# GBATZOLIS/conditional_score_diffusion

Hardware: AMD Instinct MI355X
Metric: images/sec for 1000-step PC sampling, ddpm_paired_SR3 score net of celebA_SR3_160 (BASELINE configs[1]), 160x160 (higher is better)
Workload: dtype f16x3 (every operand carried as hi + lo fp16 = 22 significand bits, 3 MFMAs per product, f32 accumulate; f32-class: the per-op test tolerance is the f32 kernel's, network error 1.9e-6 vs the reference); 1 GPU; BASELINE configs[1]: celebA_SR3_160 (ddpm_paired_SR3, nf=96, ch_mult (1,1,2,2,3,3), attn 20/10/5), 1000-step PC (reverse_diffusion + langevin, snr 0.15), batch 64 per GPU, random-init weights, synthetic LR inputs; images_per_gpu=64, global_batch=64, noise=on-device Philox4x32-10, precision_mode=fp16x3

## Files before the change

conditional_score_diffusion_amd/_lib.py:

```python
import ctypes
import os
import subprocess
import sys

_HERE = os.path.dirname(os.path.abspath(__file__))
LIB_PATH = os.environ.get('CSD_LIB_PATH', os.path.join(_HERE, 'libcsd_hip.so'))
CSRC = os.path.join(_HERE, 'csrc')

MAX_LEVELS = 8
MAX_ATTN = 8

ACT_IDS = {'none': 0, 'swish': 1, 'relu': 2, 'lrelu': 3, 'elu': 4}
PREC_IDS = {'fp32': 0, 'f32': 0, 'fp16x3': 1, 'fp16': 2, 'fp16f8': 3}


class UNetConfig(ctypes.Structure):
    _fields_ = [('arch', ctypes.c_int32), ('nf', ctypes.c_int32), ('n_levels', ctypes.c_int32),
                ('ch_mult', ctypes.c_int32 * MAX_LEVELS), ('num_res_blocks', ctypes.c_int32),
                ('n_attn', ctypes.c_int32), ('attn_resolutions', ctypes.c_int32 * MAX_ATTN),
                ('image_size', ctypes.c_int32), ('x_channels', ctypes.c_int32),
                ('y_channels', ctypes.c_int32), ('out_channels', ctypes.c_int32),
                ('resamp_with_conv', ctypes.c_int32), ('conditional', ctypes.c_int32),
                ('centered', ctypes.c_int32), ('act', ctypes.c_int32), ('precision', ctypes.c_int32),
                ('skip_rescale', ctypes.c_int32), ('progressive', ctypes.c_int32), ('progressive_input', ctypes.c_int32),
# ... 83 lines not shown
    'csd_reverse_diffusion_step_ex': (_i, [_vp, _vp, _vp, _vp, _f, _f, _f, _f, _i, _f, _f, _i, _i64, _vp]),
    'csd_row_norms': (_i, [_vp, _vp, _i, _i64, _vp]),
    'csd_affine_noise_step': (_i, [_vp, _vp, _vp, _vp, _f, _f, _f, _i64, _vp]),
    'csd_linear': (_i, [_vp, _vp, _vp, _vp, _i, _i, _i, _i, _vp]),
    'csd_fourier_embedding': (_i, [_vp, _vp, _vp, _i, _i, _vp]),
    'csd_axpby': (_i, [_vp, _vp, _vp, _f, _f, _f, _f, _i64, _vp]),
    'csd_bias_add_nchw': (_i, [_vp, _vp, _vp, _i, _i, _i64, _i, _i, _vp]),
    'csd_randn': (_i, [_vp, _i64, _u64, _u64, _vp]),
    'csd_scale_rows': (_i, [_vp, _vp, _vp, _i, _i, _i64, _vp]),
    'csd_groupnorm_scratch_bytes': (_sz, [_i, _i, _i, _i]),
    'csd_groupnorm_act': (_i, [_vp, _vp, _vp, _vp, _i, _i, _i, _i, _i, _f, _i, _vp, _vp]),
    'csd_conv_scratch_bytes': (_sz, [_i, _i, _i, _i, _i, _i, _i]),
    'csd_conv2d': (_i, [_vp, _vp, _vp, _vp, _i, _i, _i, _i, _i, _i, _i, _i, _i, _i, _vp, _vp]),
    'csd_attention_scratch_bytes': (_sz, [_i, _i, _i, _i]),
    'csd_attention': (_i, [_vp, _vp, _vp, _vp, _i, _i, _i, _i, _vp, _vp]),
    'csd_fir_pyr_conv_scratch_bytes': (_sz, [_i, _i]),
    'csd_fir_pyr_conv': (_i, [_vp, _vp, _vp, _vp, _vp, _i, _i, _i, _i, _i, _vp, _f, _vp, _vp]),
    'csd_upfirdn2d': (_i, [_vp, _vp, _vp, _i, _i, _i, _i, _i, _i, _i, _i, _i, _i, _i, _i, _i, _i, _vp]),
    'csd_fused_bias_act': (_i, [_vp, _vp, _vp, _vp, _i64, _i, _i64, _i, _i, _f, _f, _vp]),
    'csd_nearest_up2': (_i, [_vp, _vp, _i, _i, _i, _i, _vp]),
    'csd_timestep_embedding': (_i, [_vp, _vp, _i, _i, _vp]),
    'csd_conv_wgrad_scratch_bytes': (_sz, [_i, _i, _i, _i, _i, _i, _i, _i]),
    'csd_conv2d_wgrad': (_i, [_vp, _vp, _vp, _i, _i, _i, _i, _i, _i, _i, _i, _i, _vp, _vp]),
    'csd_groupnorm_act_backward': (_i, [_vp, _vp, _vp, _vp, _vp, _vp, _vp, _i, _i, _i, _i, _i, _f, _i, _vp]),
    'csd_attention_backward_scratch_bytes': (_sz, [_i, _i, _i, _i]),
    'csd_attention_backward': (_i, [_vp, _vp, _vp, _vp, _vp, _vp, _vp, _i, _i, _i, _i, _vp, _vp]),
    'csd_bgemm': (_i, [_vp, _vp, _vp, _i, _i, _i, _i64, _i64, _i64, _i64, _i64, _i64, _i, _i64, _i64, _i64, _f, _vp]),
    'csd_sum_inner': (_i, [_vp, _vp, _i64, _i64, _vp]),
    'csd_sum_rows': (_i, [_vp, _vp, _i, _i, _vp]),
    'csd_act': (_i, [_vp, _vp, _vp, _i, _i64, _vp]),
    'csd_mul': (_i, [_vp, _vp, _vp, _i64, _vp]),
    'csd_conv3x3_block_scratch_bytes': (_sz, [_i, _i]),
    'csd_conv3x3_block': (_i, [_vp, _vp, _vp, _vp, _vp, _vp, _vp, _i, _vp, _f, _vp, _vp, _i, _i, _i, _i, _i, _i, _i, _vp, _vp]),
    'csd_conv2d_ex': (_i, [_vp, _vp, _vp, _vp, _i, _i, _i, _i, _i, _i, _i, _i, _i, _i, _i, _vp, _vp]),
    'csd_conv2d_wgrad_ex': (_i, [_vp, _vp, _vp, _i, _i, _i, _i, _i, _i, _i, _i, _i, _i, _vp, _vp]),
    'csd_groupnorm_nhwc_scratch_bytes': (_sz, [_i, _i, _i]),
    'csd_groupnorm_act_nhwc': (_i, [_vp, _vp, _vp, _vp, _vp, _vp, _i, _i, _i, _i, _f, _i, _vp, _vp]),
    'csd_groupnorm_act_backward_nhwc': (_i, [_vp, _vp, _vp, _vp, _vp, _vp, _vp, _vp, _vp, _i, _i, _i, _i, _i, _i, _vp, _vp]),
    'csd_bias_add_nhwc': (_i, [_vp, _vp, _vp, _i, _i, _i, _vp]),
    'csd_sum_pixels_scratch_bytes': (_sz, [_i, _i, _i]),
    'csd_sum_pixels_nhwc': (_i, [_vp, _vp, _i, _i, _i, _vp, _vp]),
    'csd_zero_insert_odd_nhwc': (_i, [_vp, _vp, _i, _i, _i, _i, _vp]),
    'csd_sumpool2_nhwc': (_i, [_vp, _vp, _i, _i, _i, _i, _vp]),
    'csd_attention_nhwc': (_i, [_vp, _vp, _i, _i, _i, _vp]),
    'csd_attention_nhwc_prec': (_i, [_vp, _vp, _i, _i, _i, _i, _vp]),
    'csd_attention_backward_nhwc': (_i, [_vp, _vp, _vp, _i, _i, _i, _vp, _vp]),
    'csd_adam_step': (_i, [_vp, _vp, _vp, _vp, _vp, _vp, _i64, _i, _f, _f, _f, _f, _f, _f, _f, _vp]),
    'csd_global_norm_scratch_bytes': (_sz, []),
    'csd_global_norm': (_i, [_vp, _vp, _i64, _vp, _vp]),
    'csd_ema_update': (_i, [_vp, _vp, _i64, _f, _vp]),
    'csd_dropout': (_i, [_vp, _vp, _vp, _f, _u64, _u64, _i64, _vp]),
    'csd_pf_ode_state': (_i, [_vp, _vp, _vp, _vp, _i, _i64, _vp]),
    'csd_pf_ode_scratch_bytes': (_sz, [_i, _i64]),
    'csd_pf_ode_rhs': (_i, [_vp, _vp, _vp, _vp, _i64, _vp, _vp, _vp, _i, _i64, _vp, _vp]),
}


def lib():
    global _lib
    if _lib is None:
        if not os.path.exists(LIB_PATH):
            raise RuntimeError(
                'libcsd_hip.so not found at %s - run `python -c "import __graft_entry__ as g; g.build()"` '
                '(or `make -C %s`). There is no CPU fallback.' % (LIB_PATH, CSRC))
        l = ctypes.CDLL(LIB_PATH)
        for name, (res, args) in SIGNATURES.items():
# ... 63 lines not shown
```

conditional_score_diffusion_amd/csrc/common.h:

```cpp
#pragma once
#include <hip/hip_runtime.h>
#include <stdint.h>
#include <stdio.h>
#include <string>

#include "../../include/csd.h"

#ifdef CSD_TUNE
#define CSD_TUNE_ENV(name) getenv(name)
#else
#define CSD_TUNE_ENV(name) (static_cast<const char*>(nullptr))
#endif

namespace csd {

void set_error(const char* fmt, ...);
const char* get_error();

#define CSD_CHECK_HIP(expr)                                                         \
  do {                                                                              \
    hipError_t _e = (expr);                                                         \
    if (_e != hipSuccess) {                                                         \
      csd::set_error("%s:%d: %s -> %s", __FILE__, __LINE__, #expr, hipGetErrorString(_e)); \
      return CSD_ERR_HIP;                                                           \
// ... 113 lines not shown
int conv_pack_weight(const ConvPlan& p, const float* w, int layout, int cin_src, int cout_src, int cout_off,
                     float* wpack, hipStream_t s);
int conv_launch(const ConvPlan& p, const ConvArgs& a, hipStream_t s);

bool conv16_supported(const ConvPlan& p);
int conv16_kcs(int ns, int cin);
int conv16_plan_tiles(ConvPlan* p, int ns, int kcs = 1, bool lc = false);
size_t conv16_packed_bytes(const ConvPlan& p, int ns);
int conv16_pack_weight(const ConvPlan& p, int ns, const float* w, int layout, int cin_src, int cout_src,
                       int cout_off, void* wpack, hipStream_t s);
int conv16_launch(const ConvPlan& p, int ns, const ConvArgs& a, hipStream_t s, bool in16 = false);
bool conv16q_supported(const ConvPlan& p, int ns);
size_t conv16q_packed_bytes(const ConvPlan& p, int ns);
int conv16q_pack_weight(const ConvPlan& p, int ns, const float* w, int layout, int cin_src, int cout_src, int cout_off,
                        void* wpack, hipStream_t s);
int conv16q_plan_tiles(ConvPlan* p, int ns);
bool conv16q_up4_supported(const ConvPlan& p, int ns);
bool conv16q_up4_stats_ok(const ConvPlan& p);
size_t conv16q_up4_packed_bytes(const ConvPlan& p, int ns);
int conv16q_pack_weight_up4(const ConvPlan& p, int ns, const float* w, void* wpack, hipStream_t s);
int conv16q_launch(const ConvPlan& p, int ns, const ConvArgs& a, hipStream_t s, bool raw = false);
bool convff_supported(const ConvPlan& p, int ns);
size_t convff_packed_bytes(const ConvPlan& p, int ns);
int convff_pack_weight(const ConvPlan& p, int ns, const float* w, int layout, int cin_src, int cout_src, int cout_off,
                       void* wpack, hipStream_t s);
int convff_plan_tiles(ConvPlan* p, int ns);
bool convff_pipelined(const ConvPlan& p, int ns);
int convff_launch(const ConvPlan& p, int ns, const ConvArgs& a, hipStream_t s);
bool pw16_supported(const ConvPlan& p, int ns);
size_t pw16_packed_bytes(const ConvPlan& p, int ns);
int pw16_pack_weight(const ConvPlan& p, int ns, const float* w, int layout, int cin_src, int cout_src, int cout_off,
                     void* wpack, hipStream_t s);
int pw16_launch(const ConvPlan& p, int ns, const ConvArgs& a, hipStream_t s);
bool pw16_taps_supported(int cin, int cout, int ns);
int pw16_taps_cout(int cout);
int pw16_pack_weight_taps(const ConvPlan& p, int ns, const float* w, int cout, void* wpack, hipStream_t s);
int tapsum_launch(const float* part, const float* bias, const float* res, float* out, int B, int H, int W, int cout, int nchw,
                  float out_scale, hipStream_t s);
bool stem_supported(int Cx, int Cy, int Cout, int S, int ns);
size_t stem_packed_bytes(int Cout, int ns);
int stem_pack_weight(const float* w, int Cin, int Cout, int ns, void* wpack, hipStream_t s);
int stem_tiles_per_image(int S);
int stem_launch(const float* x, const float* y, const float* y_noise, float y_sigma, const void* wpack, const float* bias, float* out,
                double* stats, int B, int Cx, int Cy, int Cout, int S, int centered, int ns, hipStream_t s);
int gn_fused16_groups(int HW, int C0, int C1, int G);
int gn_fused16_launch(const float* src0, const float* src1, int C0, int C1, const float* gamma, const float* beta, float eps,
                      void* hi, void* lo, int B, int HW, int G, int act, hipStream_t s, int f8, float* nscale = nullptr,
                      float* nshift = nullptr);
int gn_apply16_launch(const float* src0, const float* src1, int C0, int C1, const float* nscale, const float* nshift,
                      void* hi, void* lo, int B, int HW, int act, hipStream_t s, int f8 = 0);
static inline int precision_ns(int precision) {
  return (precision == CSD_PREC_F16X3 || precision == CSD_PREC_F16F8) ? 2 : (precision == CSD_PREC_F16 ? 1 : 0);
}

struct GNPlan {
  int B, HW, C0, C1, G, nchunk;
};
size_t gn_partial_bytes(const GNPlan& p);
int gn_plan(GNPlan* p, int B, int HW, int C0, int C1, int G);
int gn_stats_launch(const GNPlan& p, const float* src0, const float* src1, double* partial,
                    hipStream_t s, int per_channel = 0);
int gn_finalize_launch(const GNPlan& p, const double* partial, const float* gamma, const float* beta,
                       float eps, float* nscale, float* nshift, hipStream_t s, float* rs = nullptr, float* ms = nullptr);
int gn_finalize_tiles_launch(const double* p0, int tpi0, int C0, const double* p1, int tpi1, int C1, int B, int HW, int G,
                             const float* gamma, const float* beta, float eps, float* nscale, float* nshift,
                             hipStream_t s);
// ... 78 lines not shown
```

conditional_score_diffusion_amd/csrc/conv_pw16.hip:

```cpp
#include <stdlib.h>
#include <string.h>

#include "common.h"

namespace csd {

typedef _Float16 half8_t __attribute__((ext_vector_type(8)));
typedef float floatx4 __attribute__((ext_vector_type(4)));
typedef float v4f_t __attribute__((ext_vector_type(4)));
typedef unsigned int uint4_t __attribute__((ext_vector_type(4)));

#define PW_THREADS 256
#define PW_NTL 6
#define PW_WSCALE 256.0f
#ifndef PW_DEPTH
#define PW_DEPTH 2
#endif

struct PwKArgs {
  ConvArgs a;
  int C0, C1, Cout;
  int npix;
  int hw;
  int ks;
  int ntiles;
};

__device__ __forceinline__ float4 pw_gload4(const float* p) {
  const v4f_t v = *(const __attribute__((address_space(1))) v4f_t*)(p);
  return make_float4(v.x, v.y, v.z, v.w);
}

template <int NS, int MTP, int OCC>
__global__ __launch_bounds__(PW_THREADS, OCC) void pw16_kernel(const float* __restrict__ g_src0,
                                                          const float* __restrict__ g_src1,
                                                          const char* __restrict__ g_wpack, const PwKArgs k) {
  extern __shared__ __attribute__((aligned(16))) char smem[];
  constexpr int WPIX = MTP * 16;
  constexpr int TPIX = 4 * WPIX;
  const int tid = threadIdx.x;
  const int lane = tid & 63;
  const int wave = tid >> 6;
  const int l16 = lane & 15;
  const int kq = lane >> 4;
  const int ng = blockIdx.y;
  const int Cin = k.C0 + k.C1;

  const int wbytes = k.ks * PW_NTL * NS * 1024;
  float* const lds_bias = reinterpret_cast<float*>(smem + wbytes);
  const int col_base = ng * (PW_NTL * 16) + kq * 4;

  const int nt_mine = (k.ntiles - (int)blockIdx.x + (int)gridDim.x - 1) / (int)gridDim.x;
  const int total = nt_mine * k.ks;
  const bool has_norm = k.a.nscale != nullptr;
  const bool has_res = k.a.res != nullptr;
  const bool has_act = k.a.act == CSD_ACT_SWISH;
  const int ntl = min(PW_NTL, (k.Cout - (int)blockIdx.y * (PW_NTL * 16) + 15) / 16);

  constexpr int D = MTP == 1 ? 4 : PW_DEPTH;
  float4 raw[D][MTP][2];
  constexpr bool PFN = MTP == 1;
  float4 nsc[PFN ? D : 1][MTP][2], nsh[PFN ? D : 1][MTP][2];
  floatx4 acc[MTP][PW_NTL];
#pragma unroll
  for (int j = 0; j < MTP; ++j)
#pragma unroll
    for (int nt = 0; nt < PW_NTL; ++nt) acc[j][nt] = floatx4{0.f, 0.f, 0.f, 0.f};

  int l_tile = blockIdx.x, l_kk = 0, l_it = 0;
  int c_tile = blockIdx.x, c_kk = 0;

  auto issue = [&](float4 (&dst)[MTP][2], float4 (&dsc)[MTP][2], float4 (&dsh)[MTP][2]) {
    if (l_it < total) {
      const int kb = l_kk * 32;
      const bool s1 = kb >= k.C0;
      const float* src = s1 ? g_src1 : g_src0;
      const int C = s1 ? k.C1 : k.C0;
      const int ch = (s1 ? kb - k.C0 : kb) + kq * 8;
#pragma unroll
      for (int j = 0; j < MTP; ++j) {
        int p = l_tile * TPIX + wave * WPIX + j * 16 + l16;
        p = p < k.npix ? p : k.npix - 1;
        const float* q = src + (size_t)p * C + ch;
        dst[j][0] = pw_gload4(q);
        dst[j][1] = pw_gload4(q + 4);
        if (PFN && has_norm) {
          const size_t row = (size_t)(p / k.hw) * Cin + l_kk * 32 + kq * 8;
          dsc[j][0] = pw_gload4(k.a.nscale + row); dsc[j][1] = pw_gload4(k.a.nscale + row + 4);
          dsh[j][0] = pw_gload4(k.a.nshift + row); dsh[j][1] = pw_gload4(k.a.nshift + row + 4);
        }
      }
      ++l_it;
      if (++l_kk == k.ks) { l_kk = 0; l_tile += gridDim.x; }
    }
  };

#pragma unroll
  for (int u = 0; u < D; ++u) issue(raw[u], nsc[PFN ? u : 0], nsh[PFN ? u : 0]);

  wg_copy_to_lds<PW_THREADS, 9>(smem, g_wpack + (size_t)ng * wbytes, wbytes, tid);
  if (tid < PW_NTL * 16) {
    const int c = ng * (PW_NTL * 16) + tid;
    lds_bias[tid] = (k.a.bias && c < k.Cout) ? k.a.bias[c] : 0.f;
  }
  __syncthreads();

  for (int it = 0; it < total; it += D) {
#pragma unroll
    for (int u = 0; u < D; ++u) {
      if (it + u < total) {
        half8_t bh[MTP], bl[MTP];
#pragma unroll
        for (int j = 0; j < MTP; ++j) {
          float v[8] = {raw[u][j][0].x, raw[u][j][0].y, raw[u][j][0].z, raw[u][j][0].w,
                        raw[u][j][1].x, raw[u][j][1].y, raw[u][j][1].z, raw[u][j][1].w};
          if (has_norm) {
            float4 s0, s1, h0, h1;
            if constexpr (PFN) {
              s0 = nsc[u][j][0]; s1 = nsc[u][j][1]; h0 = nsh[u][j][0]; h1 = nsh[u][j][1];
            } else {
              int p = c_tile * TPIX + wave * WPIX + j * 16 + l16;
              p = p < k.npix ? p : k.npix - 1;
              const size_t row = (size_t)(p / k.hw) * Cin + c_kk * 32 + kq * 8;
              s0 = pw_gload4(k.a.nscale + row); s1 = pw_gload4(k.a.nscale + row + 4);
              h0 = pw_gload4(k.a.nshift + row); h1 = pw_gload4(k.a.nshift + row + 4);
            }
            const float sc[8] = {s0.x, s0.y, s0.z, s0.w, s1.x, s1.y, s1.z, s1.w};
            const float sh[8] = {h0.x, h0.y, h0.z, h0.w, h1.x, h1.y, h1.z, h1.w};
#pragma unroll
            for (int q = 0; q < 8; ++q) v[q] = fmaf(v[q], sc[q], sh[q]);
            if (has_act) {
#pragma unroll
              for (int q = 0; q < 8; ++q) v[q] = v[q] * __builtin_amdgcn_rcpf(1.0f + __expf(-v[q]));
            }
          }
#pragma unroll
          for (int q = 0; q < 8; ++q) {
            const _Float16 hi = (_Float16)v[q];
            bh[j][q] = hi;
            if (NS == 2) bl[j][q] = (_Float16)(v[q] - (float)hi);
          }
        }
        issue(raw[u], nsc[PFN ? u : 0], nsh[PFN ? u : 0]);
        const char* wk = smem + (size_t)c_kk * PW_NTL * NS * 1024 + lane * 16;
#pragma unroll
        for (int nt = 0; nt < PW_NTL; ++nt) {
          if (nt >= ntl) continue;
          const half8_t wh = *reinterpret_cast<const half8_t*>(wk + (nt * NS) * 1024);
          half8_t wl;
          if (NS == 2) wl = *reinterpret_cast<const half8_t*>(wk + (nt * NS + 1) * 1024);
#pragma unroll
          for (int j = 0; j < MTP; ++j) {
            if (NS == 2) {
              acc[j][nt] = __builtin_amdgcn_mfma_f32_16x16x32_f16(wl, bh[j], acc[j][nt], 0, 0, 0);
              acc[j][nt] = __builtin_amdgcn_mfma_f32_16x16x32_f16(wh, bl[j], acc[j][nt], 0, 0, 0);
            }
            acc[j][nt] = __builtin_amdgcn_mfma_f32_16x16x32_f16(wh, bh[j], acc[j][nt], 0, 0, 0);
          }
        }
        if (++c_kk == k.ks) {
          constexpr unsigned OOB = 0x80000000u;
          constexpr int RSRC_FLAGS = 0x00020000;
          const size_t p_base = (size_t)c_tile * TPIX + wave * WPIX;
          const int left = k.npix - (int)p_base;
          const __amdgpu_buffer_rsrc_t out_r = __builtin_amdgcn_make_buffer_rsrc(
              k.a.out + p_base * k.a.out_stride + k.a.out_coff, 0, OOB, RSRC_FLAGS);
          const __amdgpu_buffer_rsrc_t res_r = __builtin_amdgcn_make_buffer_rsrc(
              const_cast<float*>(has_res ? k.a.res + p_base * k.Cout : k.a.out), 0, OOB, RSRC_FLAGS);
          const float unscale = 1.0f / PW_WSCALE;
#pragma unroll
          for (int j = 0; j < MTP; ++j) {
            const int pl = j * 16 + l16;
            const bool pv = pl < left;
            uint4_t rv[PW_NTL];
#pragma unroll
            for (int nt = 0; nt < PW_NTL; ++nt) {
              const int col0 = col_base + nt * 16;
              const unsigned off = (pv && has_res && col0 < k.Cout) ? (unsigned)(pl * k.Cout + col0) * 4u : OOB;
              rv[nt] = __builtin_amdgcn_raw_buffer_load_b128(res_r, off, 0, 0);
            }
#pragma unroll
            for (int nt = 0; nt < PW_NTL; ++nt) {
              const int col0 = col_base + nt * 16;
              const float4 b = *reinterpret_cast<const float4*>(lds_bias + nt * 16 + kq * 4);
              uint4_t ov;
              ov.x = __float_as_uint(((acc[j][nt][0] * unscale + b.x) + __uint_as_float(rv[nt].x)) * k.a.out_scale);
              ov.y = __float_as_uint(((acc[j][nt][1] * unscale + b.y) + __uint_as_float(rv[nt].y)) * k.a.out_scale);
              ov.z = __float_as_uint(((acc[j][nt][2] * unscale + b.z) + __uint_as_float(rv[nt].z)) * k.a.out_scale);
              ov.w = __float_as_uint(((acc[j][nt][3] * unscale + b.w) + __uint_as_float(rv[nt].w)) * k.a.out_scale);
              const unsigned off = (pv && col0 < k.Cout) ? (unsigned)(pl * k.a.out_stride + col0) * 4u : OOB;
              __builtin_amdgcn_raw_buffer_store_b128(ov, out_r, off, 0, 0);
              acc[j][nt] = floatx4{0.f, 0.f, 0.f, 0.f};
            }
          }
          c_kk = 0;
          c_tile += gridDim.x;
        }
      }
    }
  }
}

static size_t pw16_w_bytes(const ConvPlan& p, int ns) { return (size_t)((p.C0 + p.C1) / 32) * PW_NTL * ns * 1024; }
static size_t pw16_lds_bytes(const ConvPlan& p, int ns) { return pw16_w_bytes(p, ns) + PW_NTL * 16 * sizeof(float); }

bool pw16_supported(const ConvPlan& p, int ns) {
  return p.taps == 1 && p.stride == 1 && p.up == 0 && p.C0 > 0 && p.C0 % 32 == 0 && p.C1 % 32 == 0 && p.Cout % 4 == 0 &&
         (ns == 1 || ns == 2) && pw16_lds_bytes(p, ns) <= 150 * 1024;
}

size_t pw16_packed_bytes(const ConvPlan& p, int ns) {
  const int n_groups = cdiv(p.Cout, PW_NTL * 16);
  return (size_t)n_groups * pw16_w_bytes(p, ns);
}

__global__ void pw16_pack_kernel(const float* __restrict__ w, _Float16* __restrict__ wpack, int layout, int cin_src,
                                 int cout_src, int cout_off, int ks, int ns, int cout_pad) {
  const size_t idx = (size_t)blockIdx.x * blockDim.x + threadIdx.x;
  const int cin_tot = ks * 32;
  const int t_lo = cout_off / 16, t_hi = (cout_off + cout_src + 15) / 16;
  if (idx >= (size_t)(t_hi - t_lo) * 16 * cin_tot) return;
  const int cp = t_lo * 16 + (int)(idx / cin_tot);
  const int cin = (int)(idx % cin_tot);
  const int cout = cp - cout_off;
  if (cp >= cout_pad || cout < 0 || cout >= cout_src || cin >= cin_src) return;
  const float v = ((layout == 0) ? w[(size_t)cout * cin_src + cin] : w[(size_t)cin * cout_src + cout]) * PW_WSCALE;
  const int ng = cp / (PW_NTL * 16), nt = (cp % (PW_NTL * 16)) / 16, r = cp % 16;
  const int kk = cin / 32, kq = (cin % 32) / 8, q = cin % 8;
  const int lane = kq * 16 + r;
// ... 103 lines not shown
                  float out_scale, hipStream_t s) {
  const int cp = pw16_taps_cout(cout);
  const dim3 grid(cdiv(W, 16), cdiv(H, 16), B), block(256);
  const size_t lds = (size_t)324 * cp * sizeof(float);
  switch (cout) {
#define CSD_TS_CASE(CO)                                                                                                              \
  case CO: {                                                                                                                         \
    static bool attr_set = false;                                                                                                    \
    if (!attr_set && lds > 64 * 1024) {                               \
      CSD_CHECK_HIP(hipFuncSetAttribute(reinterpret_cast<const void*>(tapsum_kernel<CO>), hipFuncAttributeMaxDynamicSharedMemorySize, \
                                        160 * 1024));                                                                               \
      attr_set = true;                                                                                                               \
    }                                                                                                                                \
    hipLaunchKernelGGL(tapsum_kernel<CO>, grid, block, lds, s, part, bias, res, out, H, W, cp, nchw, out_scale);                     \
    break;                                                                                                                           \
  }
    CSD_TS_CASE(1) CSD_TS_CASE(2) CSD_TS_CASE(3) CSD_TS_CASE(4) CSD_TS_CASE(5) CSD_TS_CASE(6)
#undef CSD_TS_CASE
    default:
      set_error("tapsum: %d output channels not instantiated", cout);
      return CSD_ERR_INVALID;
  }
  CSD_LAUNCH_CHECK();
  return CSD_OK;
}

bool pw16_taps_supported(int cin, int cout, int ns) {
  ConvPlan p;
  memset(&p, 0, sizeof(p));
  p.taps = 1; p.stride = 1; p.C0 = cin; p.Cout = pw16_taps_cout(cout);
  return cout >= 1 && cout <= 6 && pw16_supported(p, ns) && !CSD_TUNE_ENV("CSD_NO_TAPSUM");
}

template <int NS, int MTP, int OCC>
static int pw16_launch_t(const PwKArgs& k, const ConvPlan& p, hipStream_t s) {
  auto kern = pw16_kernel<NS, MTP, OCC>;
  const size_t lds = pw16_lds_bytes(p, NS);
  static size_t attr_lds = 0;
  if (lds > attr_lds) {
    if (hipFuncSetAttribute(reinterpret_cast<const void*>(kern), hipFuncAttributeMaxDynamicSharedMemorySize, 160 * 1024) !=
        hipSuccess) {
      set_error("pw16: cannot raise the dynamic LDS limit");
      return CSD_ERR_HIP;
    }
    attr_lds = 160 * 1024;
  }
  const int n_groups = cdiv(p.Cout, PW_NTL * 16);
  int gx = (OCC * 256) / n_groups;
  if (gx < 1) gx = 1;
  if (gx > k.ntiles) gx = k.ntiles;
  hipLaunchKernelGGL(kern, dim3(gx, n_groups), dim3(PW_THREADS), lds, s, k.a.src0, k.a.src1,
                     reinterpret_cast<const char*>(k.a.wpack), k);
  CSD_LAUNCH_CHECK();
  return CSD_OK;
}

int pw16_launch(const ConvPlan& p, int ns, const ConvArgs& a, hipStream_t s) {
  CSD_REQUIRE(pw16_supported(p, ns), "pw16: unsupported layer (taps %d C0 %d C1 %d Cout %d)", p.taps, p.C0, p.C1, p.Cout);
  CSD_REQUIRE(!a.temb && !a.out_nchw && (a.act == CSD_ACT_NONE || (a.act == CSD_ACT_SWISH && a.nscale)),
              "pw16: temb / NCHW output / an activation without a GroupNorm are not supported");
  PwKArgs k;
  k.a = a;
  k.C0 = p.C0; k.C1 = p.C1; k.Cout = p.Cout;
  k.npix = p.B * p.OH * p.OW;
  k.hw = p.OH * p.OW;
  k.ks = (p.C0 + p.C1) / 32;
  const bool big = cdiv(k.npix, 128) >= 768;
  k.ntiles = cdiv(k.npix, big ? 128 : 64);
  if (ns == 2) return big ? pw16_launch_t<2, 2, 2>(k, p, s) : pw16_launch_t<2, 1, 2>(k, p, s);
  return big ? pw16_launch_t<1, 2, 3>(k, p, s) : pw16_launch_t<1, 1, 2>(k, p, s);
}

}
```

conditional_score_diffusion_amd/csrc/ops_api.hip:

```cpp
#include <stdlib.h>
#include <string.h>

#include "common.h"

using namespace csd;

namespace {
inline int ceil8(int v) { return (v + 7) / 8 * 8; }
inline int ceil16(int v) { return (v + 15) / 16 * 16; }
inline size_t al64(size_t v) { return (v + 63) / 64 * 64; }
}

extern "C" size_t csd_groupnorm_scratch_bytes(int B, int C, int H, int W) {
  GNPlan g;
  if (gn_plan(&g, B, H * W, C, 0, 1)) return 0;
  const size_t t = (size_t)B * H * W * C;
  return (2 * al64(t) + 2 * al64((size_t)B * C)) * sizeof(float) + gn_partial_bytes(g) * 64 + 1024;
}

extern "C" int csd_groupnorm_act(const float* x, const float* gamma, const float* beta, float* y, int B, int C,
                                 int H, int W, int groups, float eps, int act, void* scratch, void* stream) {
  CSD_REQUIRE(x && gamma && beta && y && scratch, "groupnorm: null argument");
  hipStream_t s = (hipStream_t)stream;
  GNPlan g;
// ... 189 lines not shown

extern "C" size_t csd_conv3x3_block_scratch_bytes(int Cin, int Cout) {
  ConvPlan p;
  memset(&p, 0, sizeof(p));
  p.C0 = Cin; p.Cout = Cout;
  return convff_packed_bytes(p, 2) / 3 * 4 + 4096 + 256;
}

extern "C" int csd_conv3x3_block(const float* x0, const float* x1, const float* weight, const float* bias, const float* nscale,
                                 const float* nshift, const float* temb, int temb_stride, const float* res, float out_scale,
                                 float* y, double* stats, int B, int C0, int C1, int Cout, int H, int W, int precision,
                                 void* scratch, void* stream) {
  CSD_REQUIRE(x0 && weight && y && scratch, "conv3x3_block: null argument");
  CSD_REQUIRE(precision == CSD_PREC_F16X3 || precision == CSD_PREC_F16 || precision == CSD_PREC_F16F8,
              "conv3x3_block: precision must be fp16x3, fp16 or fp16f8");
  hipStream_t s = (hipStream_t)stream;
  const int ns = precision == CSD_PREC_F16F8 ? 3 : precision_ns(precision);
  ConvPlan p;
  memset(&p, 0, sizeof(p));
  p.B = B; p.IH = p.OH = H; p.IW = p.OW = W; p.C0 = C0; p.C1 = C1; p.Cout = Cout; p.taps = 9; p.stride = 1; p.pad = 1; p.up = 0;
  CSD_REQUIRE(convff_supported(p, ns), "conv3x3_block: unsupported shape (C %d+%d -> %d, %dx%d)", C0, C1, Cout, H, W);
  int rc = convff_plan_tiles(&p, ns);
  if (rc) return rc;
  void* wpack = reinterpret_cast<void*>((reinterpret_cast<uintptr_t>(scratch) + 255) & ~(uintptr_t)255);
  if ((rc = convff_pack_weight(p, ns, weight, 0, C0 + C1, Cout, 0, wpack, s))) return rc;
  ConvArgs a;
  memset(&a, 0, sizeof(a));
  a.src0 = x0; a.src1 = x1; a.wpack = static_cast<const float*>(wpack); a.bias = bias; a.temb = temb; a.res = res;
  a.nscale = nscale; a.nshift = nshift; a.out = y; a.temb_stride = temb_stride; a.out_stride = Cout; a.out_coff = 0;
  a.out_nchw = 0; a.act = CSD_ACT_SWISH; a.out_scale = out_scale; a.stats = stats; a.dbg = nullptr;
  return convff_launch(p, ns, a, s);
}

extern "C" size_t csd_attention_scratch_bytes(int B, int C, int H, int W) {
  const size_t L = (size_t)H * W;
  return (al64((size_t)B * L * 3 * C) + al64((size_t)B * L * C)) * sizeof(float) + 1024;
}

extern "C" int csd_attention(const float* q, const float* k, const float* v, float* out, int B, int C, int H, int W,
                             void* scratch, void* stream) {
  CSD_REQUIRE(q && k && v && out && scratch, "attention: null argument");
  hipStream_t s = (hipStream_t)stream;
  const int L = H * W;
  float* f = static_cast<float*>(scratch);
  float* qkv = f; f += al64((size_t)B * L * 3 * C);
  float* oh = f;
  int rc;
  if ((rc = nchw_to_nhwc_launch(q, qkv, B, C, L, C, 3 * C, s))) return rc;
  if ((rc = nchw_to_nhwc_launch(k, qkv + C, B, C, L, C, 3 * C, s))) return rc;
  if ((rc = nchw_to_nhwc_launch(v, qkv + 2 * C, B, C, L, C, 3 * C, s))) return rc;
  if ((rc = attention_launch(qkv, 3 * C, oh, B, L, C, s))) return rc;
  return nhwc_to_nchw_launch(oh, out, B, C, L, C, s);
}

extern "C" int csd_linear(const float* in, const float* weight, const float* bias, float* out, int B, int K, int N,
                          int act_in, void* stream) {
  CSD_REQUIRE(in && weight && out && B > 0 && K > 0 && N > 0, "linear: bad arguments");
  return linear_launch(in, weight, bias, out, B, K, N, act_in, (hipStream_t)stream);
}

extern "C" int csd_fourier_embedding(const float* t, const float* W, float* out, int B, int E, void* stream) {
  CSD_REQUIRE(t && W && out && B > 0 && E > 0, "fourier_embedding: bad arguments");
  return fourier_embedding_launch(t, W, out, B, E, (hipStream_t)stream);
}

extern "C" int csd_axpby(const float* a, const float* b, float* out, float alpha, float beta, float gamma, float post,
// ... 11 lines not shown
```

conditional_score_diffusion_amd/ops.py:

```python
import ctypes

import torch

from . import _lib
from ._lib import check, current_stream, lib, ptr, require_gpu_tensor


def _scratch(nbytes, device):
    return torch.empty(max(int(nbytes), 256), dtype=torch.uint8, device=device)


def _c(t, name):
    require_gpu_tensor(t, name)
    return t.contiguous()


def groupnorm_act(x, gamma, beta, groups=32, eps=1e-6, act='none'):
    x, gamma, beta = _c(x, 'x'), _c(gamma, 'gamma'), _c(beta, 'beta')
    B, C, H, W = x.shape
    y = torch.empty_like(x)
    sc = _scratch(lib().csd_groupnorm_scratch_bytes(B, C, H, W), x.device)
    check(lib().csd_groupnorm_act(ptr(x), ptr(gamma), ptr(beta), ptr(y), B, C, H, W, groups, eps,
                                  _lib.ACT_IDS[act], ptr(sc), current_stream(x.device)), 'groupnorm_act')
    return y


def conv2d(x, weight, bias=None, stride=1, downsample_pad=False, up2=False, precision='fp32'):
    x, weight = _c(x, 'x'), _c(weight, 'weight')
    if bias is not None:
        bias = _c(bias, 'bias')
    B, Cin, H, W = x.shape
    Cout, Cin_w, kh, kw = weight.shape
    if Cin_w != Cin or kh != kw:
        raise RuntimeError('conv2d: weight %s does not match input channels %d' % (tuple(weight.shape), Cin))
    OH = (H * (2 if up2 else 1)) // stride
    OW = (W * (2 if up2 else 1)) // stride
    y = torch.empty(B, Cout, OH, OW, dtype=torch.float32, device=x.device)
    sc = _scratch(lib().csd_conv_scratch_bytes(B, Cin, Cout, H, W, kh, int(up2)), x.device)
    check(lib().csd_conv2d(ptr(x), ptr(weight), ptr(bias), ptr(y), B, Cin, Cout, H, W, kh, stride,
                           1 if downsample_pad else 0, int(up2), _lib.PREC_IDS[precision], ptr(sc),
                           current_stream(x.device)), 'conv2d')
    return y


def fir_pyr_conv(x, weight, bias=None, res=None, fir_kernel=(1, 3, 3, 1), out_scale=1.0):
    import ctypes
    x, weight = _c(x, 'x'), _c(weight, 'weight')
    B, H, W, Cin = x.shape
    Cout = weight.shape[0]
    if H != W or H % 2 or tuple(weight.shape[1:]) != (Cin, 3, 3):
        raise RuntimeError('fir_pyr_conv: x %s / weight %s do not match' % (tuple(x.shape), tuple(weight.shape)))
    if bias is not None:
        bias = _c(bias, 'bias')
        if tuple(bias.shape) != (Cout,):
            raise RuntimeError('fir_pyr_conv: bias %s is not [Cout] = [%d]' % (tuple(bias.shape), Cout))
    if res is not None:
        res = _c(res, 'res')
        if tuple(res.shape) != (B, H // 2, H // 2, Cout):
            raise RuntimeError('fir_pyr_conv: res %s is not [B, H/2, H/2, Cout]' % (tuple(res.shape),))
    if any(t is not None and t.device != x.device for t in (weight, bias, res)):
        raise RuntimeError('fir_pyr_conv: x, weight, bias and res must be on one device')
    taps = None
    if fir_kernel is not None:
        if len(fir_kernel) != 4:
            raise NotImplementedError('fir_pyr_conv: 4-tap FIR kernels only')
        taps = (ctypes.c_float * 4)(*[float(v) for v in fir_kernel])
    y = torch.empty(B, H // 2, H // 2, Cout, dtype=torch.float32, device=x.device)
    sc = _scratch(lib().csd_fir_pyr_conv_scratch_bytes(Cin, Cout), x.device)
    check(lib().csd_fir_pyr_conv(ptr(x), ptr(weight), ptr(bias), ptr(res), ptr(y), B, Cin, Cout, H, Cin,
                                 ctypes.cast(taps, ctypes.c_void_p) if taps is not None else None, float(out_scale), ptr(sc),
                                 current_stream(x.device)), 'fir_pyr_conv')
    return y


# ... 236 lines not shown
```

include/csd.h:

```cpp
#ifndef CSD_H_
#define CSD_H_

#include <stddef.h>
#include <stdint.h>

#ifdef __cplusplus
extern "C" {
#endif

typedef enum csd_status {
  CSD_OK = 0,
  CSD_ERR_INVALID = -1,
  CSD_ERR_HIP = -2,
  CSD_ERR_STATE = -3,
  CSD_ERR_NOT_FOUND = -4,
  CSD_ERR_WORKSPACE = -5,
  CSD_ERR_NONFINITE = -6
} csd_status;

enum { CSD_ACT_NONE = 0, CSD_ACT_SWISH = 1, CSD_ACT_RELU = 2, CSD_ACT_LRELU = 3, CSD_ACT_ELU = 4 };

enum {
  CSD_PREC_F32 = 0,
  CSD_PREC_F16X3 = 1,
// ... 172 lines not shown
                      int bias_stride, int act, void* stream);

size_t csd_conv_wgrad_scratch_bytes(int B, int Cin, int Cout, int H, int W, int ksize, int stride, int up2);
int csd_conv2d_wgrad(const float* x, const float* dy, float* dw, int B, int Cin, int Cout, int H, int W, int ksize,
                     int stride, int pad_mode, int up2, void* scratch, void* stream);
int csd_groupnorm_act_backward(const float* x, const float* gamma, const float* beta, const float* dy, float* dx,
                               float* dgamma_rows, float* dbeta_rows, int B, int C, int H, int W, int groups, float eps,
                               int act, void* stream);
size_t csd_attention_backward_scratch_bytes(int B, int C, int H, int W);
int csd_attention_backward(const float* q, const float* k, const float* v, const float* dout, float* dq, float* dk,
                           float* dv, int B, int C, int H, int W, void* scratch, void* stream);
int csd_bgemm(const float* A, const float* B, float* C, int M, int N, int K, int64_t sam, int64_t sak, int64_t sbk,
              int64_t sbn, int64_t scm, int64_t scn, int batch, int64_t za, int64_t zb, int64_t zc, float alpha,
              void* stream);
int csd_sum_inner(const float* x, float* out, int64_t rows, int64_t inner, void* stream);
int csd_sum_rows(const float* x, float* out, int R, int C, void* stream);
int csd_act(const float* x, const float* dy, float* out, int act, int64_t n, void* stream);
int csd_mul(const float* a, const float* b, float* out, int64_t n, void* stream);
int csd_dropout(const float* x, float* out, float* mask, float p, uint64_t seed, uint64_t stream_id, int64_t n,
                void* stream);

int csd_adam_step(float* param, const float* grad, float* exp_avg, float* exp_avg_sq, float* ema,
                  const float* grad_norm, int64_t n, int step, float lr, float beta1, float beta2, float eps,
                  float weight_decay, float max_norm, float ema_decay, void* stream);
size_t csd_global_norm_scratch_bytes(void);
int csd_global_norm(const float* a, float* out, int64_t n, void* scratch, void* stream);
int csd_ema_update(float* ema, const float* param, int64_t n, float decay, void* stream);

size_t csd_conv3x3_block_scratch_bytes(int Cin, int Cout);
int csd_conv3x3_block(const float* x0, const float* x1, const float* weight, const float* bias, const float* nscale,
                      const float* nshift, const float* temb, int temb_stride, const float* res, float out_scale, float* y,
                      double* stats, int B, int C0, int C1, int Cout, int H, int W, int precision, void* scratch, void* stream);

int csd_conv2d_ex(const float* x, const float* weight, const float* bias, float* y, int B, int Cin, int Cout, int H, int W,
                  int ksize, int stride, int pad_mode, int up2, int precision, int layout, void* scratch, void* stream);
int csd_conv2d_wgrad_ex(const float* x, const float* dy, float* dw, int B, int Cin, int Cout, int H, int W, int ksize,
                        int stride, int pad_mode, int up2, int layout, void* scratch, void* stream);
size_t csd_groupnorm_nhwc_scratch_bytes(int B, int C, int HW);
int csd_groupnorm_act_nhwc(const float* x, const float* gamma, const float* beta, float* y, float* rs, float* ms, int B,
                           int C, int HW, int groups, float eps, int act, void* scratch, void* stream);
int csd_groupnorm_act_backward_nhwc(const float* x, const float* gamma, const float* beta, const float* rs, const float* ms,
                                    const float* dy, float* dx, float* dgamma_rows, float* dbeta_rows, int row_stride, int B, int C,
                                    int HW, int groups, int act, void* scratch, void* stream);
int csd_bias_add_nhwc(const float* x, const float* bias, float* out, int B, int HW, int C, void* stream);
size_t csd_sum_pixels_scratch_bytes(int B, int HW, int C);
int csd_sum_pixels_nhwc(const float* x, float* out, int B, int HW, int C, void* scratch, void* stream);
int csd_zero_insert_odd_nhwc(const float* dy, float* z, int B, int h, int w, int C, void* stream);
int csd_sumpool2_nhwc(const float* in, float* out, int B, int h, int w, int C, void* stream);
int csd_attention_nhwc(const float* qkv, float* out, int B, int L, int C, void* stream);
int csd_attention_nhwc_prec(const float* qkv, float* out, int B, int L, int C, int precision, void* stream);
int csd_attention_backward_nhwc(const float* qkv, const float* dout, float* dqkv, int B, int L, int C, void* scratch,
                                void* stream);

size_t csd_unet_train_workspace_bytes(csd_unet* net, int B, float dropout_p);
int csd_unet_train_forward(csd_unet* net, const float* const* params, void* workspace, size_t workspace_bytes, const float* x,
                           const float* y, const float* labels, float* out, int B, float dropout_p, uint64_t dropout_seed,
                           uint64_t call_index, void* stream);
int csd_unet_backward(csd_unet* net, const float* const* params, float* const* grads, void* workspace, size_t workspace_bytes,
                      const float* d_out, int B, uint64_t call_index, void* stream);
int csd_unet_backward_ex(csd_unet* net, const float* const* params, float* const* grads, float* d_x, void* workspace,
                         size_t workspace_bytes, const float* d_out, int B, uint64_t call_index, void* stream);
int csd_unet_train_release(csd_unet* net, const void* workspace);
int csd_unet_train_release_call(csd_unet* net, const void* workspace, uint64_t call_index);
int csd_unet_backward_marks(csd_unet* net, const int* first_module, void* const* events, int n);
uint64_t csd_unet_backward_marks_epoch(csd_unet* net);
void* csd_event_create(void);
// ... 14 lines not shown
```

Before: 1.595 images/sec.

## Specialize pw16 fp16x3 big-tile kernel: deeper prefetch, bound-free loop, paired block mapping

Measured after the change: 1.606 images/sec, median of 6. Within noise of the previous version (+0.7%).

```diff
diff --git a/conditional_score_diffusion_amd/_lib.py b/conditional_score_diffusion_amd/_lib.py
--- a/conditional_score_diffusion_amd/_lib.py
+++ b/conditional_score_diffusion_amd/_lib.py
@@ -139,6 +139,9 @@
     'csd_mul': (_i, [_vp, _vp, _vp, _i64, _vp]),
     'csd_conv3x3_block_scratch_bytes': (_sz, [_i, _i]),
     'csd_conv3x3_block': (_i, [_vp, _vp, _vp, _vp, _vp, _vp, _vp, _i, _vp, _f, _vp, _vp, _i, _i, _i, _i, _i, _i, _i, _vp, _vp]),
+    'csd_conv1x1_block_tile_pixels': (_i, [_i, _i, _i]),
+    'csd_conv1x1_block_scratch_bytes': (_sz, [_i, _i, _i, _i, _i, _i]),
+    'csd_conv1x1_block': (_i, [_vp, _vp, _vp, _vp, _vp, _vp, _vp, _f, _vp, _i, _i, _i, _i, _i, _i, _i, _i, _vp, _vp]),
     'csd_conv2d_ex': (_i, [_vp, _vp, _vp, _vp, _i, _i, _i, _i, _i, _i, _i, _i, _i, _i, _i, _vp, _vp]),
     'csd_conv2d_wgrad_ex': (_i, [_vp, _vp, _vp, _i, _i, _i, _i, _i, _i, _i, _i, _i, _i, _vp, _vp]),
     'csd_groupnorm_nhwc_scratch_bytes': (_sz, [_i, _i, _i]),
diff --git a/conditional_score_diffusion_amd/csrc/common.h b/conditional_score_diffusion_amd/csrc/common.h
--- a/conditional_score_diffusion_amd/csrc/common.h
+++ b/conditional_score_diffusion_amd/csrc/common.h
@@ -169,6 +169,7 @@
 int pw16_pack_weight(const ConvPlan& p, int ns, const float* w, int layout, int cin_src, int cout_src, int cout_off,
                      void* wpack, hipStream_t s);
 int pw16_launch(const ConvPlan& p, int ns, const ConvArgs& a, hipStream_t s);
+int pw16_tile_pixels(int npix);
 bool pw16_taps_supported(int cin, int cout, int ns);
 int pw16_taps_cout(int cout);
 int pw16_pack_weight_taps(const ConvPlan& p, int ns, const float* w, int cout, void* wpack, hipStream_t s);
diff --git a/conditional_score_diffusion_amd/csrc/conv_pw16.hip b/conditional_score_diffusion_amd/csrc/conv_pw16.hip
--- a/conditional_score_diffusion_amd/csrc/conv_pw16.hip
+++ b/conditional_score_diffusion_amd/csrc/conv_pw16.hip
@@ -1,5 +1,7 @@
 #include <stdlib.h>
 #include <string.h>
+
+#include <type_traits>
 
 #include "common.h"
 
@@ -15,6 +17,12 @@
 #define PW_WSCALE 256.0f
 #ifndef PW_DEPTH
 #define PW_DEPTH 2
+#endif
+#ifndef PW_DEPTH1
+#define PW_DEPTH1 4
+#endif
+#ifndef PW_ABL
+#define PW_ABL 0
 #endif
 
 struct PwKArgs {
@@ -24,14 +32,15 @@
   int hw;
   int ks;
   int ntiles;
+  int gx;
+  int pair;
 };
 
 __device__ __forceinline__ float4 pw_gload4(const float* p) {
   const v4f_t v = *(const __attribute__((address_space(1))) v4f_t*)(p);
   return make_float4(v.x, v.y, v.z, v.w);
 }
-
-template <int NS, int MTP, int OCC>
+template <int NS, int MTP, int OCC, int DP = PW_DEPTH, bool HN = false>
 __global__ __launch_bounds__(PW_THREADS, OCC) void pw16_kernel(const float* __restrict__ g_src0,
                                                           const float* __restrict__ g_src1,
                                                           const char* __restrict__ g_wpack, const PwKArgs k) {
@@ -43,23 +52,29 @@
   const int wave = tid >> 6;
   const int l16 = lane & 15;
   const int kq = lane >> 4;
-  const int ng = blockIdx.y;
+  int ng = blockIdx.y, bx = blockIdx.x;
+  if (k.pair) {
+    const int lin = (int)blockIdx.y * k.gx + (int)blockIdx.x, q = lin >> 3;
+    ng = q & 1;
+    bx = (q >> 1) * 8 + (lin & 7);
+  }
   const int Cin = k.C0 + k.C1;
 
   const int wbytes = k.ks * PW_NTL * NS * 1024;
   float* const lds_bias = reinterpret_cast<float*>(smem + wbytes);
   const int col_base = ng * (PW_NTL * 16) + kq * 4;
 
-  const int nt_mine = (k.ntiles - (int)blockIdx.x + (int)gridDim.x - 1) / (int)gridDim.x;
+  const int nt_mine = (k.ntiles - bx + k.gx - 1) / k.gx;
   const int total = nt_mine * k.ks;
-  const bool has_norm = k.a.nscale != nullptr;
+  constexpr bool FREE = MTP == 2 && NS == 2;
+  const bool has_norm = FREE ? HN : k.a.nscale != nullptr;
   const bool has_res = k.a.res != nullptr;
   const bool has_act = k.a.act == CSD_ACT_SWISH;
-  const int ntl = min(PW_NTL, (k.Cout - (int)blockIdx.y * (PW_NTL * 16) + 15) / 16);
-
-  constexpr int D = MTP == 1 ? 4 : PW_DEPTH;
+  const int ntl = min(PW_NTL, (k.Cout - ng * (PW_NTL * 16) + 15) / 16);
+
+  constexpr int D = MTP == 1 ? 4 : DP;
   float4 raw[D][MTP][2];
-  constexpr bool PFN = MTP == 1;
+  constexpr bool PFN = MTP == 1 || HN;
   float4 nsc[PFN ? D : 1][MTP][2], nsh[PFN ? D : 1][MTP][2];
   floatx4 acc[MTP][PW_NTL];
 #pragma unroll
@@ -67,11 +82,11 @@
 #pragma unroll
     for (int nt = 0; nt < PW_NTL; ++nt) acc[j][nt] = floatx4{0.f, 0.f, 0.f, 0.f};
 
-  int l_tile = blockIdx.x, l_kk = 0, l_it = 0;
-  int c_tile = blockIdx.x, c_kk = 0;
+  int l_tile = bx, l_kk = 0, l_it = 0;
+  int c_tile = bx, c_kk = 0;
 
   auto issue = [&](float4 (&dst)[MTP][2], float4 (&dsc)[MTP][2], float4 (&dsh)[MTP][2]) {
-    if (l_it < total) {
+    if (FREE || l_it < total) {
       const int kb = l_kk * 32;
       const bool s1 = kb >= k.C0;
       const float* src = s1 ? g_src1 : g_src0;
@@ -91,7 +106,7 @@
         }
       }
       ++l_it;
-      if (++l_kk == k.ks) { l_kk = 0; l_tile += gridDim.x; }
+      if (++l_kk == k.ks) { l_kk = 0; l_tile += k.gx; }
     }
   };
 
@@ -105,10 +120,49 @@
   }
   __syncthreads();
 
+  auto epilogue = [&](auto with_res) {
+    constexpr bool HR = decltype(with_res)::value;
+    constexpr unsigned OOB = 0x80000000u;
+    constexpr int RSRC_FLAGS = 0x00020000;
+    const size_t p_base = (size_t)c_tile * TPIX + wave * WPIX;
+    const int left = k.npix - (int)p_base;
+    const __amdgpu_buffer_rsrc_t out_r = __builtin_amdgcn_make_buffer_rsrc(
+        k.a.out + p_base * k.a.out_stride + k.a.out_coff, 0, OOB, RSRC_FLAGS);
+    const __amdgpu_buffer_rsrc_t res_r = __builtin_amdgcn_make_buffer_rsrc(
+        const_cast<float*>(has_res ? k.a.res + p_base * k.Cout : k.a.out), 0, OOB, RSRC_FLAGS);
+    const float unscale = 1.0f / PW_WSCALE;
+#pragma unroll
+    for (int j = 0; j < MTP; ++j) {
+      const int pl = j * 16 + l16;
+      const bool pv = pl < left;
+      uint4_t rv[PW_NTL];
+#pragma unroll
+      for (int nt = 0; nt < PW_NTL; ++nt) {
+        const int col0 = col_base + nt * 16;
+        const unsigned off = (pv && has_res && col0 < k.Cout) ? (unsigned)(pl * k.Cout + col0) * 4u : OOB;
+        if constexpr (HR) rv[nt] = __builtin_amdgcn_raw_buffer_load_b128(res_r, off, 0, 0);
+        else rv[nt] = uint4_t{0u, 0u, 0u, 0u};
+      }
+#pragma unroll
+      for (int nt = 0; nt < PW_NTL; ++nt) {
+        const int col0 = col_base + nt * 16;
+        const float4 b = *reinterpret_cast<const float4*>(lds_bias + nt * 16 + kq * 4);
+        uint4_t ov;
+        ov.x = __float_as_uint(((acc[j][nt][0] * unscale + b.x) + __uint_as_float(rv[nt].x)) * k.a.out_scale);
+        ov.y = __float_as_uint(((acc[j][nt][1] * unscale + b.y) + __uint_as_float(rv[nt].y)) * k.a.out_scale);
+        ov.z = __float_as_uint(((acc[j][nt][2] * unscale + b.z) + __uint_as_float(rv[nt].z)) * k.a.out_scale);
+        ov.w = __float_as_uint(((acc[j][nt][3] * unscale + b.w) + __uint_as_float(rv[nt].w)) * k.a.out_scale);
+        const unsigned off = (pv && col0 < k.Cout && !(PW_ABL & 2)) ? (unsigned)(pl * k.a.out_stride + col0) * 4u : OOB;
+        __builtin_amdgcn_raw_buffer_store_b128(ov, out_r, off, 0, 0);
+        acc[j][nt] = floatx4{0.f, 0.f, 0.f, 0.f};
+      }
+    }
+  };
+
   for (int it = 0; it < total; it += D) {
 #pragma unroll
     for (int u = 0; u < D; ++u) {
-      if (it + u < total) {
+      if (FREE || it + u < total) {
         half8_t bh[MTP], bl[MTP];
 #pragma unroll
         for (int j = 0; j < MTP; ++j) {
@@ -131,7 +185,8 @@
             for (int q = 0; q < 8; ++q) v[q] = fmaf(v[q], sc[q], sh[q]);
             if (has_act) {
 #pragma unroll
-              for (int q = 0; q < 8; ++q) v[q] = v[q] * __builtin_amdgcn_rcpf(1.0f + __expf(-v[q]));
+              for (int q = 0; q < 8; ++q)
+                v[q] = (PW_ABL & 1) ? v[q] * (v[q] * 0.7f) : v[q] * __builtin_amdgcn_rcpf(1.0f + __expf(-v[q]));
             }
           }
 #pragma unroll
@@ -151,6 +206,7 @@
           if (NS == 2) wl = *reinterpret_cast<const half8_t*>(wk + (nt * NS + 1) * 1024);
 #pragma unroll
           for (int j = 0; j < MTP; ++j) {
+            if (PW_ABL & 4) { acc[j][nt][0] += (float)wh[0] + (float)bh[j][0] + (NS == 2 ? (float)wl[0] + (float)bl[j][0] : 0.f); continue; }
             if (NS == 2) {
               acc[j][nt] = __builtin_amdgcn_mfma_f32_16x16x32_f16(wl, bh[j], acc[j][nt], 0, 0, 0);
               acc[j][nt] = __builtin_amdgcn_mfma_f32_16x16x32_f16(wh, bl[j], acc[j][nt], 0, 0, 0);
@@ -159,42 +215,10 @@
           }
         }
         if (++c_kk == k.ks) {
-          constexpr unsigned OOB = 0x80000000u;
-          constexpr int RSRC_FLAGS = 0x00020000;
-          const size_t p_base = (size_t)c_tile * TPIX + wave * WPIX;
-          const int left = k.npix - (int)p_base;
-          const __amdgpu_buffer_rsrc_t out_r = __builtin_amdgcn_make_buffer_rsrc(
-              k.a.out + p_base * k.a.out_stride + k.a.out_coff, 0, OOB, RSRC_FLAGS);
-          const __amdgpu_buffer_rsrc_t res_r = __builtin_amdgcn_make_buffer_rsrc(
-              const_cast<float*>(has_res ? k.a.res + p_base * k.Cout : k.a.out), 0, OOB, RSRC_FLAGS);
-          const float unscale = 1.0f / PW_WSCALE;
-#pragma unroll
-          for (int j = 0; j < MTP; ++j) {
-            const int pl = j * 16 + l16;
-            const bool pv = pl < left;
-            uint4_t rv[PW_NTL];
-#pragma unroll
-            for (int nt = 0; nt < PW_NTL; ++nt) {
-              const int col0 = col_base + nt * 16;
-              const unsigned off = (pv && has_res && col0 < k.Cout) ? (unsigned)(pl * k.Cout + col0) * 4u : OOB;
-              rv[nt] = __builtin_amdgcn_raw_buffer_load_b128(res_r, off, 0, 0);
-            }
-#pragma unroll
-            for (int nt = 0; nt < PW_NTL; ++nt) {
-              const int col0 = col_base + nt * 16;
-              const float4 b = *reinterpret_cast<const float4*>(lds_bias + nt * 16 + kq * 4);
-              uint4_t ov;
-              ov.x = __float_as_uint(((acc[j][nt][0] * unscale + b.x) + __uint_as_float(rv[nt].x)) * k.a.out_scale);
-              ov.y = __float_as_uint(((acc[j][nt][1] * unscale + b.y) + __uint_as_float(rv[nt].y)) * k.a.out_scale);
-              ov.z = __float_as_uint(((acc[j][nt][2] * unscale + b.z) + __uint_as_float(rv[nt].z)) * k.a.out_scale);
-              ov.w = __float_as_uint(((acc[j][nt][3] * unscale + b.w) + __uint_as_float(rv[nt].w)) * k.a.out_scale);
-              const unsigned off = (pv && col0 < k.Cout) ? (unsigned)(pl * k.a.out_stride + col0) * 4u : OOB;
-              __builtin_amdgcn_raw_buffer_store_b128(ov, out_r, off, 0, 0);
-              acc[j][nt] = floatx4{0.f, 0.f, 0.f, 0.f};
-            }
-          }
+          if (!FREE || has_res) epilogue(std::true_type{});
+          else epilogue(std::false_type{});
           c_kk = 0;
-          c_tile += gridDim.x;
+          c_tile += k.gx;
         }
       }
     }
@@ -364,9 +388,9 @@
   return cout >= 1 && cout <= 6 && pw16_supported(p, ns) && !CSD_TUNE_ENV("CSD_NO_TAPSUM");
 }
 
-template <int NS, int MTP, int OCC>
-static int pw16_launch_t(const PwKArgs& k, const ConvPlan& p, hipStream_t s) {
-  auto kern = pw16_kernel<NS, MTP, OCC>;
+template <int NS, int MTP, int OCC, int DP = PW_DEPTH, bool HN = false>
+static int pw16_launch_t(PwKArgs& k, const ConvPlan& p, hipStream_t s) {
+  auto kern = pw16_kernel<NS, MTP, OCC, DP, HN>;
   const size_t lds = pw16_lds_bytes(p, NS);
   static size_t attr_lds = 0;
   if (lds > attr_lds) {
@@ -378,14 +402,19 @@
     attr_lds = 160 * 1024;
   }
   const int n_groups = cdiv(p.Cout, PW_NTL * 16);
-  int gx = (OCC * 256) / n_groups;
+  const int per_cu = (MTP == 2 && 2 * lds > 160 * 1024) ? 1 : OCC;
+  int gx = (per_cu * 256) / n_groups;
   if (gx < 1) gx = 1;
   if (gx > k.ntiles) gx = k.ntiles;
+  k.gx = gx;
+  k.pair = MTP == 2 && n_groups == 2 && gx % 8 == 0;
   hipLaunchKernelGGL(kern, dim3(gx, n_groups), dim3(PW_THREADS), lds, s, k.a.src0, k.a.src1,
                      reinterpret_cast<const char*>(k.a.wpack), k);
   CSD_LAUNCH_CHECK();
   return CSD_OK;
 }
+
+int pw16_tile_pixels(int npix) { return cdiv(npix, 128) >= 768 ? 128 : 64; }
 
 int pw16_launch(const ConvPlan& p, int ns, const ConvArgs& a, hipStream_t s) {
   CSD_REQUIRE(pw16_supported(p, ns), "pw16: unsupported layer (taps %d C0 %d C1 %d Cout %d)", p.taps, p.C0, p.C1, p.Cout);
@@ -397,9 +426,15 @@
   k.npix = p.B * p.OH * p.OW;
   k.hw = p.OH * p.OW;
   k.ks = (p.C0 + p.C1) / 32;
-  const bool big = cdiv(k.npix, 128) >= 768;
+  k.pair = 0;
+  const bool big = pw16_tile_pixels(k.npix) == 128;
   k.ntiles = cdiv(k.npix, big ? 128 : 64);
-  if (ns == 2) return big ? pw16_launch_t<2, 2, 2>(k, p, s) : pw16_launch_t<2, 1, 2>(k, p, s);
+  if (ns == 2 && big) {
+    if (a.nscale) return pw16_launch_t<2, 2, 2, PW_DEPTH, true>(k, p, s);
+    if (2 * pw16_lds_bytes(p, 2) > 160 * 1024) return pw16_launch_t<2, 2, 2, PW_DEPTH1>(k, p, s);
+    return pw16_launch_t<2, 2, 2>(k, p, s);
+  }
+  if (ns == 2) return pw16_launch_t<2, 1, 2>(k, p, s);
   return big ? pw16_launch_t<1, 2, 3>(k, p, s) : pw16_launch_t<1, 1, 2>(k, p, s);
 }
 
diff --git a/conditional_score_diffusion_amd/csrc/ops_api.hip b/conditional_score_diffusion_amd/csrc/ops_api.hip
--- a/conditional_score_diffusion_amd/csrc/ops_api.hip
+++ b/conditional_score_diffusion_amd/csrc/ops_api.hip
@@ -245,6 +245,44 @@
   return convff_launch(p, ns, a, s);
 }
 
+extern "C" int csd_conv1x1_block_tile_pixels(int B, int H, int W) { return pw16_tile_pixels(B * H * W); }
+
+extern "C" size_t csd_conv1x1_block_scratch_bytes(int B, int H, int W, int Cin, int Cout, int ksize) {
+  ConvPlan p;
+  memset(&p, 0, sizeof(p));
+  p.taps = 1; p.stride = 1; p.C0 = Cin; p.Cout = ksize == 3 ? pw16_taps_cout(Cout) : Cout;
+  const size_t part = ksize == 3 ? (size_t)B * H * W * p.Cout * sizeof(float) : 0;
+  return pw16_packed_bytes(p, 2) + part + 1024;
+}
+
+extern "C" int csd_conv1x1_block(const float* x0, const float* x1, const float* weight, const float* bias, const float* nscale,
+                                 const float* nshift, const float* res, float out_scale, float* y, int B, int C0, int C1, int Cout,
+                                 int H, int W, int ksize, int precision, void* scratch, void* stream) {
+  CSD_REQUIRE(x0 && weight && y && scratch && (ksize == 1 || ksize == 3), "conv1x1_block: bad argument");
+  CSD_REQUIRE(precision == CSD_PREC_F16X3 || precision == CSD_PREC_F16, "conv1x1_block: precision must be fp16x3 or fp16");
+  CSD_REQUIRE((nscale != nullptr) == (nshift != nullptr), "conv1x1_block: scale and shift come together");
+  hipStream_t s = (hipStream_t)stream;
+  const int ns = precision_ns(precision);
+  const bool taps = ksize == 3;
+  ConvPlan p;
+  memset(&p, 0, sizeof(p));
+  p.B = B; p.IH = p.OH = H; p.IW = p.OW = W; p.C0 = C0; p.C1 = C1; p.taps = 1; p.stride = 1;
+  p.Cout = taps ? pw16_taps_cout(Cout) : Cout;
+  CSD_REQUIRE(taps ? (C1 == 0 && nscale && pw16_taps_supported(C0, Cout, ns)) : pw16_supported(p, ns),
+              "conv1x1_block: unsupported shape (C %d+%d -> %d, ksize %d)", C0, C1, Cout, ksize);
+  char* const wpack = reinterpret_cast<char*>((reinterpret_cast<uintptr_t>(scratch) + 255) & ~(uintptr_t)255);
+  float* const part = reinterpret_cast<float*>(wpack + (pw16_packed_bytes(p, ns) + 255) / 256 * 256);
+  int rc = taps ? pw16_pack_weight_taps(p, ns, weight, Cout, wpack, s) : pw16_pack_weight(p, ns, weight, 0, C0 + C1, Cout, 0, wpack, s);
+  if (rc) return rc;
+  ConvArgs a;
+  memset(&a, 0, sizeof(a));
+  a.src0 = x0; a.src1 = x1; a.wpack = reinterpret_cast<const float*>(wpack); a.bias = taps ? nullptr : bias;
+  a.res = taps ? nullptr : res; a.nscale = nscale; a.nshift = nshift; a.out = taps ? part : y; a.out_stride = p.Cout;
+  a.act = nscale ? CSD_ACT_SWISH : CSD_ACT_NONE; a.out_scale = taps ? 1.f : out_scale;
+  if ((rc = pw16_launch(p, ns, a, s))) return rc;
+  return taps ? tapsum_launch(part, bias, res, y, B, H, W, Cout, 0, out_scale, s) : CSD_OK;
+}
+
 extern "C" size_t csd_attention_scratch_bytes(int B, int C, int H, int W) {
   const size_t L = (size_t)H * W;
   return (al64((size_t)B * L * 3 * C) + al64((size_t)B * L * C)) * sizeof(float) + 1024;
diff --git a/conditional_score_diffusion_amd/ops.py b/conditional_score_diffusion_amd/ops.py
--- a/conditional_score_diffusion_amd/ops.py
+++ b/conditional_score_diffusion_amd/ops.py
@@ -40,6 +40,23 @@
     check(lib().csd_conv2d(ptr(x), ptr(weight), ptr(bias), ptr(y), B, Cin, Cout, H, W, kh, stride,
                            1 if downsample_pad else 0, int(up2), _lib.PREC_IDS[precision], ptr(sc),
                            current_stream(x.device)), 'conv2d')
+    return y
+
+
+def conv1x1_block(x0, weight, x1=None, bias=None, nscale=None, nshift=None, res=None, out_scale=1.0, precision='fp16x3'):
+    x0, weight = _c(x0, 'x0'), _c(weight, 'weight')
+    opt = [None if t is None else _c(t, n) for t, n in ((x1, 'x1'), (bias, 'bias'), (nscale, 'nscale'), (nshift, 'nshift'), (res, 'res'))]
+    x1, bias, nscale, nshift, res = opt
+    B, H, W, C0 = x0.shape
+    C1 = 0 if x1 is None else x1.shape[3]
+    Cout, ksize = weight.shape[0], (3 if weight.dim() == 4 else 1)
+    if weight.shape[1] != C0 + C1 or (x1 is not None and tuple(x1.shape[:3]) != (B, H, W)):
+        raise RuntimeError('conv1x1_block: weight %s / sources %d + %d do not match' % (tuple(weight.shape), C0, C1))
+    y = torch.empty(B, H, W, Cout, dtype=torch.float32, device=x0.device)
+    sc = _scratch(lib().csd_conv1x1_block_scratch_bytes(B, H, W, C0 + C1, Cout, ksize), x0.device)
+    check(lib().csd_conv1x1_block(ptr(x0), ptr(x1), ptr(weight), ptr(bias), ptr(nscale), ptr(nshift), ptr(res), float(out_scale),
+                                  ptr(y), B, C0, C1, Cout, H, W, ksize, _lib.PREC_IDS[precision], ptr(sc),
+                                  current_stream(x0.device)), 'conv1x1_block')
     return y
 
 
diff --git a/include/csd.h b/include/csd.h
--- a/include/csd.h
+++ b/include/csd.h
@@ -228,6 +228,12 @@
                       const float* nshift, const float* temb, int temb_stride, const float* res, float out_scale, float* y,
                       double* stats, int B, int C0, int C1, int Cout, int H, int W, int precision, void* scratch, void* stream);
 
+int csd_conv1x1_block_tile_pixels(int B, int H, int W);
+size_t csd_conv1x1_block_scratch_bytes(int B, int H, int W, int Cin, int Cout, int ksize);
+int csd_conv1x1_block(const float* x0, const float* x1, const float* weight, const float* bias, const float* nscale,
+                      const float* nshift, const float* res, float out_scale, float* y, int B, int C0, int C1, int Cout, int H,
+                      int W, int ksize, int precision, void* scratch, void* stream);
+
 int csd_conv2d_ex(const float* x, const float* weight, const float* bias, float* y, int B, int Cin, int Cout, int H, int W,
                   int ksize, int stride, int pad_mode, int up2, int precision, int layout, void* scratch, void* stream);
 int csd_conv2d_wgrad_ex(const float* x, const float* dy, float* dw, int B, int Cin, int Cout, int H, int W, int ksize,
```
